# ethz-asl/voxgraph

Measured on AMD Instinct MI355X. Metric: Mresiduals+Jacobians/s per GPU; full pose-graph solve ms (200 submaps), higher is better.
Workload: dtype f32

## Files before the change

### profiles/fuzz_esdf.py

```python
#!/usr/bin/env python3
import os
import sys

import numpy as np

ROOT = os.path.dirname(os.path.dirname(os.path.abspath(__file__)))
sys.path.insert(0, ROOT)
F = np.float32
BAR = 4e-3


def main():
    from oracle import pyoracle as orc
    from oracle import synth
    from tests.test_esdf_gpu import _check_fixed_point
    from voxgraph_amd import capi
    capi.load()
    ctx = capi.Context(0)
    n_seeds, first = int(os.environ.get("SEEDS", "100")), int(os.environ.get("FIRST", "0"))
    done, worst, worst_fp, voxels, frontier = 0, 0.0, 0.0, 0, 0
    for seed in range(first, first + n_seeds):
        rng = np.random.default_rng(seed)
        vps = int(rng.choice([8, 16]))
        vs = float(rng.choice([0.05, 0.1, 0.2]))
        dims = tuple(int(x) for x in rng.integers(1, 5, 3))
        ext = np.array(dims) * vps * vs
        c = rng.uniform(0.2, 0.8, 3) * ext
        sdf = synth.sphere_ground_sdf(tuple(c), float(rng.uniform(0.2, 0.6) * ext.min()), float(rng.uniform(0.1, 0.4) * ext[2]))
        sm = synth.make_submap(sdf, vs, vps, tuple(int(x) for x in rng.integers(-2, 2, 3)), dims, trunc=3 * vs, esdf_max=10 * vs,
                               drop_empty_blocks=bool(rng.integers(0, 2)))
        if len(sm.block_index) == 0:
            continue
        td = sm.tsdf_distance.copy()
        if rng.integers(0, 2):
            td = np.clip(td + rng.normal(0, 0.02 * vs, td.shape).astype(F), -3 * vs, 3 * vs).astype(F)
        tw = sm.tsdf_weight.copy()
        if rng.integers(0, 2):
            tw = np.where(rng.uniform(size=tw.shape) < 0.03, 0, tw).astype(F)
        max_d = float(rng.choice([2.0, 6 * vs, 12 * vs]))
        kw = dict(max_distance_m=max_d, default_distance_m=float(rng.choice([max_d, 2.0])), min_distance_m=float(rng.choice([0.2, vs, 2 * vs])))
        what = dict(seed=seed, vps=vps, vs=vs, dims=dims, blocks=len(sm.block_index), **kw)
        g = capi.Submap(ctx, 0, vs, vps, sm.block_index, td, tw, None, None)
        try:
            g.generate_esdf(capi.esdf_config(**kw))
            _, _, ed, eo = g.download_layers(vps)
            od, oo, _ = orc.esdf_from_tsdf(vs, vps, sm.block_index, td, tw, orc.esdf_config(**kw))
            assert np.array_equal(eo, oo), "observed masks"
            obs = oo.astype(bool)
            fixed = (tw >= 1e-6) & (np.abs(td) < kw["min_distance_m"])
            assert np.array_equal(ed[fixed], td[fixed]), "fixed band"
            assert np.array_equal(np.sign(ed[obs]), np.sign(td[obs])), "signs"
            if obs.any():
                a_d, a_o = np.abs(ed), np.abs(od)
                lo = kw["max_distance_m"] - BAR
                frontier_v = obs & (kw["default_distance_m"] > kw["max_distance_m"]) & ((a_d > lo) | (a_o > lo))
                assert np.all(np.minimum(a_d[frontier_v], a_o[frontier_v]) > lo - BAR), "a shell voxel on one side, an inner one on the other"
                frontier += int((frontier_v & (np.abs(ed - od) >= BAR)).sum())
                cmp_ = obs & ~frontier_v
                diff = np.abs(ed - od)[cmp_]
                assert diff.size == 0 or diff.max() < BAR, ("distance", float(diff.max()))
                assert np.all(np.abs(ed[cmp_]) <= np.abs(od[cmp_]) + 1e-6), "device above the queue's value"
                worst = max(worst, float(diff.max()) if diff.size else 0.0)
                try:
                    err, n_free = _check_fixed_point(sm.block_index, td, ed, eo, vs, vps, kw["min_distance_m"], kw["max_distance_m"],
                                                     kw["default_distance_m"])
                except ValueError:
                    err, n_free = 0.0, 0
                assert err < 1e-6, ("fixed point", err)
                worst_fp = max(worst_fp, err)
                voxels += int(obs.sum())
        except AssertionError as e:
            print("MISMATCH", what, str(e)[:300])
            return 1
        finally:
            g.destroy()
        done += 1
    print("no mismatch in %d submaps (%d observed voxels): worst |device - queue| %.2e m (bar %.1e), worst fixed-point residual %.1e; "
          "%d voxels of the shell beyond max_distance_m differ by more (default > max configurations only)" %
          (done, voxels, worst, BAR, worst_fp, frontier))
    ctx.close()
    return 0


if __name__ == "__main__":
    sys.exit(main())
```

### voxgraph_amd/csrc/vgx_context.hip

```cpp
#include <algorithm>
#include <atomic>
#include <cmath>
#include <cstring>
#include <numeric>

#include <cstdlib>

#include "vgx_internal.h"

namespace vgx {

static std::mutex g_err_mu;
static std::string g_global_error = "no error";

void set_global_error(const std::string& msg) {
  std::lock_guard<std::mutex> lk(g_err_mu);
  g_global_error = msg;
}

int set_error(vgx_ctx ctx, int code, const std::string& msg) {
  if (ctx) {
    std::lock_guard<std::mutex> lk(ctx->err_mu);
    ctx->last_error = msg;
  } else {
    set_global_error(msg);
  }
  return code;
}

template <int VPS, int LAYOUT>
__global__ __launch_bounds__(256) void brickify_kernel(
    const int32_t* __restrict__ block_index, const int32_t* __restrict__ lut,
    int3 lut_min, int3 lut_dim, const float* __restrict__ distance,
    const float* __restrict__ weight, const uint8_t* __restrict__ observed,
    float* __restrict__ bricks) {
  constexpr int CELLS = BrickLayout<VPS, LAYOUT>::cells;
  constexpr int VOX = VPS * VPS * VPS;
  const int b = blockIdx.x;
  const int bx = block_index[3 * b + 0] - lut_min.x;
  const int by = block_index[3 * b + 1] - lut_min.y;
  const int bz = block_index[3 * b + 2] - lut_min.z;
  float* out = bricks + (size_t)b * CELLS;
  for (int cell = threadIdx.x; cell < CELLS; cell += blockDim.x) {
    int cx, cy, cz;
    BrickLayout<VPS, LAYOUT>::decode(cell, cx, cy, cz);
    int ox = cx == VPS, oy = cy == VPS, oz = cz == VPS;
    int sx = bx + ox, sy = by + oy, sz = bz + oz;
    int slot = b;
    if (ox | oy | oz) {
      slot = -1;
      if (sx < lut_dim.x && sy < lut_dim.y && sz < lut_dim.z)
        slot = lut[sx + lut_dim.x * (sy + lut_dim.y * sz)];
    }
    float v = __builtin_nanf("");
    if (slot >= 0) {
      int vx = ox ? 0 : cx, vy = oy ? 0 : cy, vz = oz ? 0 : cz;
      size_t at = (size_t)slot * VOX + vx + VPS * (vy + VPS * vz);
      bool ok = weight ? (weight[at] > 0.0f) : (observed[at] != 0);
      if (ok) v = distance[at];
    }
    out[cell] = v;
  }
}

int launch_brickify(vgx_submap sm, int which) {
  vgx_ctx ctx = sm->ctx;
  const float* dist = which == 0 ? sm->d_tsdf_distance : sm->d_esdf_distance;
  const float* w = which == 0 ? sm->d_tsdf_weight.get() : nullptr;
  const uint8_t* obs = which == 0 ? nullptr : sm->d_esdf_observed.get();
  const int layout = ctx->brick_layout;
  const size_t cells = brick_cells(sm->vps, layout);
  if ((unsigned long long)sm->n_blocks * cells >= (1ull << 32))
    return set_error(ctx, VGX_ERR_UNSUPPORTED,
                     "submap too large for 32-bit brick addressing: " + std::to_string(sm->n_blocks) + " blocks x " +
                         std::to_string(cells) + " cells per brick");
  size_t bytes = (size_t)sm->n_blocks * cells * sizeof(float);
  VGX_HIP(ctx, sm->grid[which].d_bricks.alloc(bytes));
  sm->grid[which].layout = layout;
  int3 mn = make_int3(sm->lut_min[0], sm->lut_min[1], sm->lut_min[2]);
  int3 dm = make_int3(sm->lut_dim[0], sm->lut_dim[1], sm->lut_dim[2]);
  dispatch_brick(sm->vps, layout, [&](auto V, auto L) {
    hipLaunchKernelGGL((brickify_kernel<V(), L()>), dim3(sm->n_blocks), dim3(256), 0, ctx->stream, sm->d_block_index, sm->d_lut, mn, dm,
                       dist, w, obs, sm->grid[which].d_bricks);
  });
  VGX_HIP(ctx, hipGetLastError());
  sm->grid[which].present = true;
  return VGX_OK;
}

template <int VPS>
__global__ __launch_bounds__(256) void requad_kernel(const float* __restrict__ apron, float* __restrict__ quad) {
  constexpr int CA = BrickLayout<VPS, 0>::cells, CQ = BrickLayout<VPS, 1>::cells, B = VPS + 1;
  const float* in = apron + (size_t)blockIdx.x * CA;
  float* out = quad + (size_t)blockIdx.x * CQ;
  for (int i = threadIdx.x; i < CQ; i += blockDim.x) {
    int cx, cy, cz;
    BrickLayout<VPS, 1>::decode(i, cx, cy, cz);
    out[i] = in[cx + B * (cy + B * cz)];
  }
}

__global__ __launch_bounds__(64) void chunk_bounds_kernel(const float4* __restrict__ xyzd, long long n,
                                                         float4* __restrict__ bounds,
                                                         float* __restrict__ chunk_minmax) {
  const long long first = (long long)blockIdx.x * kChunkPoints;
  float mn[3] = {INFINITY, INFINITY, INFINITY}, mx[3] = {-INFINITY, -INFINITY, -INFINITY};
  for (long long i = first + threadIdx.x; i < first + kChunkPoints && i < n; i += 64) {
    float4 p = xyzd[i];
    mn[0] = fminf(mn[0], p.x); mx[0] = fmaxf(mx[0], p.x);
    mn[1] = fminf(mn[1], p.y); mx[1] = fmaxf(mx[1], p.y);
    mn[2] = fminf(mn[2], p.z); mx[2] = fmaxf(mx[2], p.z);
  }
#pragma unroll
  for (int a = 0; a < 3; ++a)
#pragma unroll
    for (int off = 32; off >= 1; off >>= 1) {
      mn[a] = fminf(mn[a], __shfl_xor(mn[a], off, 64));
      mx[a] = fmaxf(mx[a], __shfl_xor(mx[a], off, 64));
    }
  if (threadIdx.x == 0) {
    float hx = 0.5f * (mx[0] - mn[0]), hy = 0.5f * (mx[1] - mn[1]), hz = 0.5f * (mx[2] - mn[2]);
    float r = sqrtf(hx * hx + hy * hy + hz * hz) * 1.0001f + 1e-4f;
    bounds[blockIdx.x] = make_float4(0.5f * (mx[0] + mn[0]), 0.5f * (mx[1] + mn[1]),
                                     0.5f * (mx[2] + mn[2]), r);
#pragma unroll
    for (int a = 0; a < 3; ++a) {
      chunk_minmax[6 * blockIdx.x + a] = mn[a];
      chunk_minmax[6 * blockIdx.x + 3 + a] = mx[a];
    }
  }
// ... 154 lines not shown
  if (std::string(prop.gcnArchName).rfind("gfx950", 0) != 0)
    return set_error(nullptr, VGX_ERR_NO_DEVICE,
                     std::string("vgx_ctx_create: device is ") + prop.gcnArchName +
                         ", this library is built for gfx950 only");
  vgx_ctx ctx = new (std::nothrow) vgx_ctx_s();
  if (!ctx) return set_error(nullptr, VGX_ERR_NOMEM, "vgx_ctx_create: out of host memory");
  ctx->device = device;
  ctx->cu_count = prop.multiProcessorCount;
  int prio_least = 0, prio_greatest = 0;
  const bool use_prio = hipSetDevice(device) == hipSuccess &&
                        hipDeviceGetStreamPriorityRange(&prio_least, &prio_greatest) == hipSuccess;
  ctx->stream_priorities = use_prio && prio_least != prio_greatest;
  if (hipSetDevice(device) != hipSuccess ||
      hipStreamCreateWithPriority(&ctx->own_stream, hipStreamNonBlocking, ctx->stream_priorities ? prio_least : 0) != hipSuccess ||
      hipStreamCreateWithPriority(&ctx->tsdf_own_stream, hipStreamNonBlocking, ctx->stream_priorities ? prio_greatest : 0) != hipSuccess ||
      hipEventCreate(&ctx->ev_start) != hipSuccess ||
      hipEventCreate(&ctx->ev_stop) != hipSuccess ||
      hipEventCreate(&ctx->ev_tsdf_start) != hipSuccess ||
      hipEventCreate(&ctx->ev_tsdf_stop) != hipSuccess ||
      hipEventCreateWithFlags(&ctx->ev_handover, hipEventDisableTiming) != hipSuccess) {
    if (ctx->own_stream) (void)hipStreamDestroy(ctx->own_stream);
    if (ctx->tsdf_own_stream) (void)hipStreamDestroy(ctx->tsdf_own_stream);
    for (hipEvent_t ev : {ctx->ev_start, ctx->ev_stop, ctx->ev_tsdf_start, ctx->ev_tsdf_stop, ctx->ev_handover})
      if (ev) (void)hipEventDestroy(ev);
    delete ctx;
    return set_error(nullptr, VGX_ERR_HIP, "vgx_ctx_create: stream/event creation failed");
  }
  ctx->stream = ctx->own_stream;
  ctx->tsdf_stream = ctx->tsdf_own_stream;
  ctx->last_error = "no error";
  *out = ctx;
  return VGX_OK;
}

int vgx_ctx_destroy(vgx_ctx ctx) {
  if (!ctx) return VGX_ERR_INVALID;
  (void)hipSetDevice(ctx->device);
  (void)hipStreamSynchronize(ctx->stream);
  (void)hipStreamSynchronize(ctx->tsdf_stream);
  for (hipEvent_t ev : {ctx->ev_start, ctx->ev_stop, ctx->ev_tsdf_start, ctx->ev_tsdf_stop, ctx->ev_handover})
    if (ev) (void)hipEventDestroy(ev);
  for (int k = 0; k < Context::kEvalSlots; ++k) {
    Context::EvalSlot& sl = ctx->eval_slot[k];
    if (sl.stream) {
      (void)hipStreamSynchronize(sl.stream);
      (void)hipStreamDestroy(sl.stream);
    }
    if (sl.order) (void)hipEventDestroy(sl.order);
    sl.d_out.release();
    sl.d_raw.release();
    sl.h_raw.release();
    sl.h_out.release();
  }
  if (ctx->own_stream) (void)hipStreamDestroy(ctx->own_stream);
  if (ctx->tsdf_own_stream) (void)hipStreamDestroy(ctx->tsdf_own_stream);
  delete ctx;
  return VGX_OK;
}

const char* vgx_last_error(vgx_ctx ctx) {
  static thread_local std::string copy;
  if (ctx) {
    std::lock_guard<std::mutex> lk(ctx->err_mu);
    copy = ctx->last_error;
  } else {
    std::lock_guard<std::mutex> lk(g_err_mu);
    copy = g_global_error;
  }
  return copy.c_str();
}

int vgx_ctx_set_stream(vgx_ctx ctx, void* hip_stream) {
  if (!ctx) return VGX_ERR_INVALID;
  std::lock_guard<std::mutex> lk(ctx->mu);
  ctx->stream = hip_stream ? (hipStream_t)hip_stream : ctx->own_stream;
  return VGX_OK;
}

void* vgx_ctx_get_stream(vgx_ctx ctx) { return ctx ? (void*)ctx->stream : nullptr; }

int vgx_ctx_set_tsdf_stream(vgx_ctx ctx, void* hip_stream) {
  if (!ctx) return VGX_ERR_INVALID;
  std::lock_guard<std::mutex> lk(ctx->tsdf_mu);
  (void)hipSetDevice(ctx->device);
  (void)hipStreamSynchronize(ctx->tsdf_stream);
  ctx->tsdf_stream = hip_stream ? (hipStream_t)hip_stream : ctx->tsdf_own_stream;
  return VGX_OK;
}

void* vgx_ctx_get_tsdf_stream(vgx_ctx ctx) { return ctx ? (void*)ctx->tsdf_stream : nullptr; }

int vgx_ctx_set_brick_layout(vgx_ctx ctx, int32_t layout) {
  if (!ctx) return VGX_ERR_INVALID;
  if (layout != VGX_BRICKS_APRON && layout != VGX_BRICKS_QUAD)
    return set_error(ctx, VGX_ERR_INVALID, "vgx_ctx_set_brick_layout: unknown layout");
  std::lock_guard<std::mutex> lk(ctx->mu);
  ctx->brick_layout = layout;
  return VGX_OK;
}

int vgx_ctx_set_sampling_bricks(vgx_ctx ctx, int32_t mode) {
  if (!ctx) return VGX_ERR_INVALID;
  if (mode != VGX_SAMPLING_BRICKS_SAME && mode != VGX_SAMPLING_BRICKS_QUAD)
    return set_error(ctx, VGX_ERR_INVALID, "vgx_ctx_set_sampling_bricks: unknown mode");
  std::lock_guard<std::mutex> lk(ctx->mu);
  ctx->sampling_bricks = mode;
// ... 339 lines not shown
```

### voxgraph_amd/csrc/vgx_esdf.hip

```cpp
#include <cmath>
#include <vector>

#include "vgx_internal.h"

#pragma clang fp contract(off)

namespace vgx {

struct TsdfLayerDevView;

__global__ __launch_bounds__(256) void esdf_init_kernel(const float* __restrict__ tsdf_d,
                                                        const float* __restrict__ tsdf_w,
                                                        size_t n, float min_weight,
                                                        float min_distance, float default_distance,
                                                        float* __restrict__ esdf_d,
                                                        uint8_t* __restrict__ esdf_obs) {
  size_t i = (size_t)blockIdx.x * blockDim.x + threadIdx.x;
  if (i >= n) return;
  float w = tsdf_w[i], d = tsdf_d[i];
  if (w < min_weight) {
    esdf_d[i] = 0.0f;
    esdf_obs[i] = 0;
    return;
  }
  esdf_obs[i] = 1;
  if (fabsf(d) < min_distance) {
    esdf_d[i] = d;
  } else {
    float sgn = (float)((d > 0.0f) - (d < 0.0f));
    esdf_d[i] = sgn * default_distance;
  }
}

constexpr int kLocalSweeps = 6;

template <int VPS>
__global__ __launch_bounds__(256) void esdf_relax_kernel(
    const int32_t* __restrict__ block_index, const int32_t* __restrict__ lut, int3 lut_min,
    int3 lut_dim, const float* __restrict__ tsdf_d, const uint8_t* __restrict__ esdf_obs,
    float* __restrict__ esdf_d, float voxel_size, float min_distance, float max_distance,
    int* __restrict__ changed) {
  constexpr int T = VPS + 2;
  constexpr int VOX = VPS * VPS * VPS;
  __shared__ float tile[T * T * T];
  __shared__ int s_changed;
  const int b = blockIdx.x;
  const int bx = block_index[3 * b] - lut_min.x, by = block_index[3 * b + 1] - lut_min.y,
            bz = block_index[3 * b + 2] - lut_min.z;
  if (threadIdx.x == 0) s_changed = 0;
  for (int c = threadIdx.x; c < T * T * T; c += 256) {
    int tx = c % T, ty = (c / T) % T, tz = c / (T * T);
    int vx = tx - 1, vy = ty - 1, vz = tz - 1;
    int ox = vx < 0 ? -1 : (vx >= VPS ? 1 : 0), oy = vy < 0 ? -1 : (vy >= VPS ? 1 : 0),
        oz = vz < 0 ? -1 : (vz >= VPS ? 1 : 0);
    int slot = b;
    if (ox | oy | oz) {
      int sx = bx + ox, sy = by + oy, sz = bz + oz;
      slot = -1;
      if ((unsigned)sx < (unsigned)lut_dim.x && (unsigned)sy < (unsigned)lut_dim.y &&
          (unsigned)sz < (unsigned)lut_dim.z)
        slot = lut[sx + lut_dim.x * (sy + lut_dim.y * sz)];
    }
    float v = __builtin_nanf("");
    if (slot >= 0) {
      size_t at = (size_t)slot * VOX + (size_t)((vx - ox * VPS) + VPS * ((vy - oy * VPS) + VPS * (vz - oz * VPS)));
      if (esdf_obs[at]) v = esdf_d[at];
    }
    tile[c] = v;
  }
  __syncthreads();
  const float s1 = voxel_size, s2 = sqrtf(2.0f) * voxel_size, s3 = sqrtf(3.0f) * voxel_size;
  bool any_change = false;
  for (int sweep = 0; sweep < kLocalSweeps; ++sweep) {
    bool sweep_change = false;
    for (int v = threadIdx.x; v < VOX; v += 256) {
      int x = v % VPS, y = (v / VPS) % VPS, z = v / (VPS * VPS);
      int c = (x + 1) + T * ((y + 1) + T * (z + 1));
      float cur = tile[c];
      if (!(cur == cur)) continue;
      if (fabsf(tsdf_d[(size_t)b * VOX + v]) < min_distance) continue;
      float mag = fabsf(cur);
      float best = mag;
#pragma unroll
      for (int dz = -1; dz <= 1; ++dz)
#pragma unroll
        for (int dy = -1; dy <= 1; ++dy)
#pragma unroll
          for (int dx = -1; dx <= 1; ++dx) {
            if (dx == 0 && dy == 0 && dz == 0) continue;
            float n = tile[c + dx + T * (dy + T * dz)];
            int nz = (dx != 0) + (dy != 0) + (dz != 0);
            float step = nz == 1 ? s1 : (nz == 2 ? s2 : s3);
            bool same = (cur > 0.0f && n > 0.0f) || (cur < 0.0f && n < 0.0f);
            float cand = fabsf(n) + step;
            if (same && fabsf(n) < max_distance && cand < best) best = cand;
          }
      if (best < mag) {
        tile[c] = cur > 0.0f ? best : -best;
        sweep_change = true;
      }
    }
    any_change |= sweep_change;
    if (sweep_change) s_changed = 1;
    __syncthreads();
    int again = s_changed;
    __syncthreads();
    if (!again) break;
    if (threadIdx.x == 0) s_changed = 0;
    __syncthreads();
  }
  if (__syncthreads_or(any_change)) {
    for (int v = threadIdx.x; v < VOX; v += 256) {
      int x = v % VPS, y = (v / VPS) % VPS, z = v / (VPS * VPS);
      float val = tile[(x + 1) + T * ((y + 1) + T * (z + 1))];
      if (val == val) esdf_d[(size_t)b * VOX + v] = val;
    }
    if (threadIdx.x == 0) atomicExch(changed, 1);
  }
}

}

using namespace vgx;

extern "C" {

void vgx_esdf_config_default(vgx_esdf_config* c) {
  if (!c) return;
  c->max_distance_m = 2.0f;
  c->min_distance_m = 0.2f;
  c->default_distance_m = 2.0f;
  c->min_diff_m = 0.001f;
  c->min_weight = 1e-6f;
  c->num_buckets = 20;
}

int vgx_submap_generate_esdf(vgx_submap sm, const vgx_esdf_config* cfg_in, int32_t* sweeps_out) {
  if (!sm) return VGX_ERR_INVALID;
  vgx_ctx ctx = sm->ctx;
  std::lock_guard<std::mutex> lk(ctx->mu);
  vgx_esdf_config cfg;
  if (cfg_in) cfg = *cfg_in; else vgx_esdf_config_default(&cfg);
  if (sm->n_blocks > 0 && (!sm->d_tsdf_distance || !sm->d_tsdf_weight))
    return set_error(ctx, VGX_ERR_INVALID, "vgx_submap_generate_esdf: TSDF layer not resident");
  if (!(cfg.max_distance_m > 0) || !(cfg.min_distance_m >= 0) || !(cfg.default_distance_m > 0))
    return set_error(ctx, VGX_ERR_INVALID, "vgx_submap_generate_esdf: bad config");
  VGX_HIP(ctx, hipSetDevice(ctx->device));
  if (sweeps_out) *sweeps_out = 0;
  if (sm->n_blocks == 0) return VGX_OK;
  const size_t nvox = (size_t)sm->n_blocks * sm->vps * sm->vps * sm->vps;
  VGX_HIP(ctx, hipStreamSynchronize(ctx->stream));
  if (!sm->d_esdf_distance) VGX_HIP(ctx, sm->d_esdf_distance.alloc_n(nvox));
  if (!sm->d_esdf_observed) VGX_HIP(ctx, sm->d_esdf_observed.alloc_n(nvox));
  DeviceBuffer s_changed;
  VGX_HIP(ctx, s_changed.alloc(sizeof(int)));
  int* d_changed = s_changed.as<int>();
  hipLaunchKernelGGL(esdf_init_kernel, dim3((unsigned)((nvox + 255) / 256)), dim3(256), 0, ctx->stream,
                     sm->d_tsdf_distance, sm->d_tsdf_weight, nvox, cfg.min_weight, cfg.min_distance_m,
                     cfg.default_distance_m, sm->d_esdf_distance, sm->d_esdf_observed);
  int3 mn = make_int3(sm->lut_min[0], sm->lut_min[1], sm->lut_min[2]);
  int3 dm = make_int3(sm->lut_dim[0], sm->lut_dim[1], sm->lut_dim[2]);
  int passes = 0, rc = VGX_OK;
  const int max_passes = 8 + (int)std::ceil(cfg.max_distance_m / sm->voxel_size) * 2;
  while (passes < max_passes) {
    hipError_t e = hipMemsetAsync(d_changed, 0, sizeof(int), ctx->stream);
    if (e == hipSuccess) {
      if (sm->vps == 16)
        hipLaunchKernelGGL(esdf_relax_kernel<16>, dim3(sm->n_blocks), dim3(256), 0, ctx->stream,
                           sm->d_block_index, sm->d_lut, mn, dm, sm->d_tsdf_distance,
                           sm->d_esdf_observed, sm->d_esdf_distance, sm->voxel_size,
                           cfg.min_distance_m, cfg.max_distance_m, d_changed);
      else
        hipLaunchKernelGGL(esdf_relax_kernel<8>, dim3(sm->n_blocks), dim3(256), 0, ctx->stream,
                           sm->d_block_index, sm->d_lut, mn, dm, sm->d_tsdf_distance,
                           sm->d_esdf_observed, sm->d_esdf_distance, sm->voxel_size,
                           cfg.min_distance_m, cfg.max_distance_m, d_changed);
      e = hipGetLastError();
    }
    int h_changed = 0;
    if (e == hipSuccess) e = hipMemcpyAsync(&h_changed, d_changed, sizeof(int), hipMemcpyDeviceToHost, ctx->stream);
    if (e == hipSuccess) e = hipStreamSynchronize(ctx->stream);
    if (e != hipSuccess) {
      rc = set_error(ctx, VGX_ERR_HIP, std::string("vgx_submap_generate_esdf: ") + hipGetErrorString(e));
      break;
    }
    ++passes;
    if (!h_changed) break;
  }
  if (rc != VGX_OK) return rc;
  if (sweeps_out) *sweeps_out = passes;
  if (sm->grid[1].d_bricks) {
    sm->grid[1].d_bricks.release();
    sm->grid[1].present = false;
  }
  sm->grid[1].d_quad.release();
  return launch_brickify(sm, 1);
}

}
```

### voxgraph_amd/csrc/vgx_internal.h

```cpp
#ifndef VGX_INTERNAL_H_
#define VGX_INTERNAL_H_

#include <hip/hip_runtime.h>

#include <algorithm>
#include <atomic>
#include <cstdint>
#include <mutex>
#include <condition_variable>
#include <initializer_list>
#include <random>
#include <string>
#include <type_traits>
#include <utility>
#include <vector>

#include "voxgraph_amd.h"

namespace vgx {


template <int VPS, int LAYOUT>
struct BrickLayout {
  static_assert(LAYOUT == 0 || LAYOUT == 1, "apron (0) or quad (1) bricks");
// ... 207 lines not shown
  for (const DeviceBufferSize& g : group) g.buffer->release();
  hipError_t e = hipSuccess;
  for (const DeviceBufferSize& g : group)
    if (e == hipSuccess) e = g.buffer->alloc(g.bytes);
  if (e != hipSuccess)
    for (const DeviceBufferSize& g : group) g.buffer->release();
  return e;
}

template <class Call>
hipError_t temp_bytes(Call& call, size_t* bytes) {
  *bytes = 0;
  return call(nullptr, *bytes);
}
template <class Call>
hipError_t run_with_temp(DeviceBuffer& tmp, Call& call) {
  size_t bytes = 0;
  hipError_t e = temp_bytes(call, &bytes);
  if (e == hipSuccess) e = tmp.reserve(bytes, 8);
  if (e == hipSuccess) e = call(tmp.p, bytes);
  return e;
}

struct Context {
  int device = 0;
  hipStream_t own_stream = nullptr;
  hipStream_t stream = nullptr;
  hipEvent_t ev_start = nullptr, ev_stop = nullptr;
  std::mutex mu;
  hipStream_t tsdf_own_stream = nullptr;
  hipStream_t tsdf_stream = nullptr;
  bool stream_priorities = false;
  std::atomic<int> tsdf_integrators{0};
  hipEvent_t ev_tsdf_start = nullptr, ev_tsdf_stop = nullptr, ev_handover = nullptr;
  std::mutex tsdf_mu;
  std::mutex err_mu;
  std::string last_error;
  int cu_count = 256;
  int brick_layout = 0;
  int sampling_bricks = 1;
  struct EvalSlot {
    hipStream_t stream = nullptr;
    hipEvent_t order = nullptr;
    DeviceBuffer d_out;
    DeviceBuffer d_raw;
    PinnedBuffer h_raw;
    PinnedBuffer h_out;
    bool busy = false;
  };
  static constexpr int kEvalSlots = 8;
  static constexpr size_t kSmallOutputBytes = 1u << 20;
  EvalSlot eval_slot[kEvalSlots];
  std::condition_variable slot_free;
};

struct Mt19937 {
  static constexpr int kN = 624;
  uint32_t mt[kN];
  uint32_t idx = kN;
  Mt19937() { seed(5489u); }
  void seed(uint32_t s) {
    mt[0] = s;
    for (int i = 1; i < kN; ++i) mt[i] = 1812433253u * (mt[i - 1] ^ (mt[i - 1] >> 30)) + (uint32_t)i;
    idx = kN;
  }
  void twist() {
    for (int k = 0; k < kN; ++k) {
      uint32_t y = (mt[k] & 0x80000000u) | (mt[(k + 1) % kN] & 0x7fffffffu);
      mt[k] = mt[(k + 397) % kN] ^ (y >> 1) ^ ((y & 1u) ? 0x9908b0dfu : 0u);
    }
    idx = 0;
  }
  uint32_t operator()() {
    if (idx >= (uint32_t)kN) twist();
    uint32_t y = mt[idx++];
    y ^= y >> 11;
    y ^= (y << 7) & 0x9d2c5680u;
    y ^= (y << 15) & 0xefc60000u;
    y ^= y >> 18;
    return y;
  }
};
static_assert(sizeof(Mt19937) == 625 * 4, "Mt19937 is copied to the device as 625 words");

struct SamplerEngine {
  Mt19937 host;
  DeviceArray<uint32_t> d_state;
  bool on_device = false;
};

struct PointSet {
  int64_t n = 0;
  uint64_t version = 0;
  DeviceArray<float4> d_xyzd;
  DeviceArray<float> d_weight;
  DeviceArray<float4> d_chunk_bounds;
  float aabb_min[3] = {0, 0, 0}, aabb_max[3] = {0, 0, 0};
  double sum_weight = 0;
  bool present = false;
  std::vector<int64_t> order;
  std::vector<int32_t> inv_order;
  std::vector<double> cumulative_weight;
  DeviceArray<double> d_cumulative;
  int32_t search_buckets = 0;
  DeviceArray<int32_t> d_search_lut;
  DeviceArray<int32_t> d_inv_order;
// ... 127 lines not shown
  return origin + ((float)idx + 0.5f) * voxel_size;
}

#define VGX_HIP(ctx, call)                                                      \
  do {                                                                          \
    hipError_t e__ = (call);                                                    \
    if (e__ != hipSuccess)                                                      \
      return vgx::set_error((ctx), VGX_ERR_HIP,                                 \
                            std::string(#call) + ": " + hipGetErrorString(e__)); \
  } while (0)

inline int alloc_error(vgx_ctx ctx, hipError_t e, const char* what) {
  (void)hipGetLastError();
  return set_error(ctx, e == hipErrorOutOfMemory ? VGX_ERR_NOMEM : VGX_ERR_HIP, std::string(what) + ": " + hipGetErrorString(e));
}

inline int upload_new(vgx_ctx ctx, DeviceBuffer& buffer, const void* src, size_t bytes) {
  buffer.release();
  if (bytes == 0) return VGX_OK;
  VGX_HIP(ctx, buffer.alloc(bytes));
  VGX_HIP(ctx, hipMemcpy(buffer.p, src, bytes, hipMemcpyHostToDevice));
  return VGX_OK;
}

struct MeshView {
  vgx_ctx ctx;
  bool holds_mesh;
  bool has_colors;
  bool per_vertex;
  int64_t n_tris;
  const float* vertices;
  const float* normals;
  const uint32_t* colors;
};
std::mutex& mesh_mutex(vgx_mesh M);
MeshView mesh_view(vgx_mesh M);

struct EvalTotals {
  double sum;
  float max_abs, min_abs;
  long long n_eval, n_ign, n_non, n_err_blocks;
};
struct EvalDevice {
  DeviceBuffer slot, has, pos, part, tot, tmp, ed, es, ebi;
};
int eval_check(const char* fn, vgx_submap gt, vgx_submap test, int32_t layer, int32_t mode, const void* details);
int eval_enqueue(vgx_submap gt, vgx_submap test, int32_t layer, int32_t mode, bool want_index, bool want_distance, bool want_set,
                 EvalDevice& D);
void eval_details(const EvalTotals& tot, vgx_voxel_evaluation_details* details);

#ifndef VGX_TOOLING_LIBRARY
int launch_brickify(vgx_submap sm, int which);
int build_block_lut(vgx_submap sm);
#else
inline int launch_brickify(vgx_submap sm, int which);
inline int build_block_lut(vgx_submap sm);
#endif
int build_chunk_bounds(vgx_ctx ctx, PointSet& ps);
void reset_point_set(PointSet& ps);
int engine_to_host(vgx_ctx ctx, SamplerEngine& e);
int engine_to_device(vgx_ctx ctx, SamplerEngine& e);
void make_pose_pack(const double ref_pose[4], const double read_pose[4], PosePack* out);
std::vector<Tile> make_tiles(int32_t constraint, int64_t n, int tile_points);
constexpr int kBlockThreads = 256;
constexpr int kPointsPerThread = 4;
constexpr int kTilePoints = kBlockThreads * kPointsPerThread;
}

extern "C" {
VGX_API int vgx_internal_set_error(vgx_ctx ctx, int code, const char* msg);
VGX_API int vgx_internal_launch_brickify(vgx_submap sm, int which);
VGX_API int vgx_internal_build_block_lut(vgx_submap sm);
}
#ifdef VGX_TOOLING_LIBRARY
namespace vgx {
inline int set_error(vgx_ctx ctx, int code, const std::string& msg) { return vgx_internal_set_error(ctx, code, msg.c_str()); }
inline int launch_brickify(vgx_submap sm, int which) { return vgx_internal_launch_brickify(sm, which); }
inline int build_block_lut(vgx_submap sm) { return vgx_internal_build_block_lut(sm); }
}
#endif

#endif
```

Before: 130,100.

## Rework ESDF relaxation with block wake marks, batched passes and column sweeps

The ESDF relaxation kernel now tracks which blocks changed and marks only them and their neighbours for the next pass, so settled blocks exit early. The host queues several passes per synchronisation and reads per-pass counts instead of syncing after every pass. The kernel also switches to per-thread z-column sweeps with register-rolled neighbour planes and integer-keyed min comparisons, and brick buffers are reused instead of reallocated. This mainly speeds up the ESDF generation path; the pose-graph residual/Jacobian metric may be largely unaffected. It adds complexity and risks subtle correctness issues in mark bookkeeping and in the float-as-uint ordering.

After: 129,800. About the same (-0.2%).

```diff
diff --git a/profiles/esdf_bench.py b/profiles/esdf_bench.py
--- /dev/null
+++ b/profiles/esdf_bench.py
@@ -0,0 +1,115 @@
+import argparse
+import hashlib
+import json
+import os
+import sys
+import time
+
+import numpy as np
+
+ROOT = os.path.dirname(os.path.dirname(os.path.abspath(__file__)))
+sys.path.insert(0, ROOT)
+
+from voxgraph_amd import capi
+
+F = np.float32
+
+
+def city256(ctx):
+    pose = [0.0, 0.0, 0.0, np.random.default_rng(2).uniform(-0.1, 0.1)]
+    return capi.Submap.synth_city(ctx, 0, 0.2, 16, (-8, -8, -4), (16, 16, 16), 0.6, 2.0, 10.0, np.array(pose), 2)
+
+
+def config2(ctx):
+    import torch
+    from harness import pipeline
+    n_az, n_el, scans, vs = 1024, 64, 20, 0.2
+    poses = pipeline.session_sensor_poses(30, scans)
+    P = poses[0].copy()
+    P[2] = 0.0
+    pts = torch.empty((n_az * n_el, 3), dtype=torch.float32, device="cuda")
+    layer = capi.TsdfLayer(ctx, vs, 16)
+    for j in (0, scans - 1):
+        layer.reserve(pipeline._inv_compose(P, poses[j])[4:7], 16.0 + 0.6 + 2 * vs)
+    integ = capi.FastTsdfIntegrator(ctx, capi.voxgraph_tsdf_config(deterministic=1), layer)
+    for j in range(scans):
+        capi.synth_city_scan(ctx, poses[j], n_az, n_el, np.deg2rad(33.2), 40.0, 2, pts.data_ptr())
+        ctx.synchronize()
+        integ.integrate_device(pipeline._inv_compose(P, poses[j]), pts.data_ptr(), None, n_az * n_el)
+    ctx.synchronize()
+    sm = capi.Submap.from_tsdf_layer(ctx, layer, 0)
+    integ.destroy()
+    layer.destroy()
+    return sm
+
+
+def config1(ctx):
+    from oracle import synth
+    ref, _ = synth.config1_pair()
+    return capi.Submap(ctx, 0, ref.voxel_size, ref.vps, ref.block_index, ref.tsdf_distance, ref.tsdf_weight, None, None)
+
+
+def layer_hash(sm, h=None):
+    _, _, ed, eo = sm.download_layers(sm.vps)
+    h = hashlib.sha256() if h is None else h
+    h.update(ed.tobytes())
+    h.update(eo.tobytes())
+    return h
+
+
+def spread(ms):
+    return {"min": round(min(ms), 4), "median": round(float(np.median(ms)), 4), "max": round(max(ms), 4)}
+
+
+def main():
+    ap = argparse.ArgumentParser()
+    ap.add_argument("--reps", type=int, default=20)
+    ap.add_argument("--fuzz", type=int, default=0)
+    ap.add_argument("--loop", type=int, default=0)
+    ap.add_argument("--sizes", nargs="+", default=["city256", "config2", "config1"])
+    args = ap.parse_args()
+    ctx = capi.Context(0)
+    if args.loop:
+        sm = city256(ctx)
+        for _ in range(args.loop):
+            sm.generate_esdf()
+        ctx.synchronize()
+        sm.destroy()
+        ctx.close()
+        return
+    res = {"library": os.path.basename(capi.LIB_PATH), "reps": args.reps, "sizes": {}}
+    for name in args.sizes:
+        sm = {"city256": city256, "config2": config2, "config1": config1}[name](ctx)
+        for _ in range(3):
+            passes = sm.generate_esdf()
+        ev, wall = [], []
+        for _ in range(args.reps):
+            ctx.synchronize()
+            t = time.perf_counter()
+            ctx.timer_start()
+            sm.generate_esdf()
+            ev.append(ctx.timer_stop())
+            wall.append((time.perf_counter() - t) * 1e3)
+        res["sizes"][name] = {"blocks": int(sm.num_blocks()), "passes": int(passes), "event_ms": spread(ev), "wall_ms": spread(wall),
+                              "sha256": layer_hash(sm).hexdigest()}
+        sm.destroy()
+    if args.fuzz:
+        from profiles.fuzz_esdf import case
+        h, n = hashlib.sha256(), 0
+        for seed in range(args.fuzz):
+            made = case(seed)
+            if made is None:
+                continue
+            d, td, tw, kw = made
+            sm = capi.Submap(ctx, 0, d.voxel_size, d.vps, d.block_index, td, tw, None, None)
+            sm.generate_esdf(capi.esdf_config(**kw))
+            layer_hash(sm, h)
+            sm.destroy()
+            n += 1
+        res["fuzz"] = {"seeds": args.fuzz, "submaps": n, "sha256": h.hexdigest()}
+    ctx.close()
+    print(json.dumps(res))
+
+
+if __name__ == "__main__":
+    main()
diff --git a/profiles/fuzz_esdf.py b/profiles/fuzz_esdf.py
--- a/profiles/fuzz_esdf.py
+++ b/profiles/fuzz_esdf.py
@@ -10,6 +10,30 @@
 BAR = 4e-3
 
 
+def case(seed):
+    from oracle import synth
+    rng = np.random.default_rng(seed)
+    vps = int(rng.choice([8, 16]))
+    vs = float(rng.choice([0.05, 0.1, 0.2]))
+    dims = tuple(int(x) for x in rng.integers(1, 5, 3))
+    ext = np.array(dims) * vps * vs
+    c = rng.uniform(0.2, 0.8, 3) * ext
+    sdf = synth.sphere_ground_sdf(tuple(c), float(rng.uniform(0.2, 0.6) * ext.min()), float(rng.uniform(0.1, 0.4) * ext[2]))
+    sm = synth.make_submap(sdf, vs, vps, tuple(int(x) for x in rng.integers(-2, 2, 3)), dims, trunc=3 * vs, esdf_max=10 * vs,
+                           drop_empty_blocks=bool(rng.integers(0, 2)))
+    if len(sm.block_index) == 0:
+        return None
+    td = sm.tsdf_distance.copy()
+    if rng.integers(0, 2):
+        td = np.clip(td + rng.normal(0, 0.02 * vs, td.shape).astype(F), -3 * vs, 3 * vs).astype(F)
+    tw = sm.tsdf_weight.copy()
+    if rng.integers(0, 2):
+        tw = np.where(rng.uniform(size=tw.shape) < 0.03, 0, tw).astype(F)
+    max_d = float(rng.choice([2.0, 6 * vs, 12 * vs]))
+    kw = dict(max_distance_m=max_d, default_distance_m=float(rng.choice([max_d, 2.0])), min_distance_m=float(rng.choice([0.2, vs, 2 * vs])))
+    return sm, td, tw, kw
+
+
 def main():
     from oracle import pyoracle as orc
     from oracle import synth
@@ -20,26 +44,12 @@
     n_seeds, first = int(os.environ.get("SEEDS", "100")), int(os.environ.get("FIRST", "0"))
     done, worst, worst_fp, voxels, frontier = 0, 0.0, 0.0, 0, 0
     for seed in range(first, first + n_seeds):
-        rng = np.random.default_rng(seed)
-        vps = int(rng.choice([8, 16]))
-        vs = float(rng.choice([0.05, 0.1, 0.2]))
-        dims = tuple(int(x) for x in rng.integers(1, 5, 3))
-        ext = np.array(dims) * vps * vs
-        c = rng.uniform(0.2, 0.8, 3) * ext
-        sdf = synth.sphere_ground_sdf(tuple(c), float(rng.uniform(0.2, 0.6) * ext.min()), float(rng.uniform(0.1, 0.4) * ext[2]))
-        sm = synth.make_submap(sdf, vs, vps, tuple(int(x) for x in rng.integers(-2, 2, 3)), dims, trunc=3 * vs, esdf_max=10 * vs,
-                               drop_empty_blocks=bool(rng.integers(0, 2)))
-        if len(sm.block_index) == 0:
+        made = case(seed)
+        if made is None:
             continue
-        td = sm.tsdf_distance.copy()
-        if rng.integers(0, 2):
-            td = np.clip(td + rng.normal(0, 0.02 * vs, td.shape).astype(F), -3 * vs, 3 * vs).astype(F)
-        tw = sm.tsdf_weight.copy()
-        if rng.integers(0, 2):
-            tw = np.where(rng.uniform(size=tw.shape) < 0.03, 0, tw).astype(F)
-        max_d = float(rng.choice([2.0, 6 * vs, 12 * vs]))
-        kw = dict(max_distance_m=max_d, default_distance_m=float(rng.choice([max_d, 2.0])), min_distance_m=float(rng.choice([0.2, vs, 2 * vs])))
-        what = dict(seed=seed, vps=vps, vs=vs, dims=dims, blocks=len(sm.block_index), **kw)
+        sm, td, tw, kw = made
+        vs, vps = sm.voxel_size, sm.vps
+        what = dict(seed=seed, vps=vps, vs=vs, blocks=len(sm.block_index), **kw)
         g = capi.Submap(ctx, 0, vs, vps, sm.block_index, td, tw, None, None)
         try:
             g.generate_esdf(capi.esdf_config(**kw))
diff --git a/voxgraph_amd/csrc/vgx_context.hip b/voxgraph_amd/csrc/vgx_context.hip
--- a/voxgraph_amd/csrc/vgx_context.hip
+++ b/voxgraph_amd/csrc/vgx_context.hip
@@ -63,19 +63,29 @@
   }
 }
 
+int reserve_bricks(vgx_submap sm, int which) {
+  vgx_ctx ctx = sm->ctx;
+  const size_t cells = brick_cells(sm->vps, ctx->brick_layout);
+  if ((unsigned long long)sm->n_blocks * cells >= (1ull << 32))
+    return set_error(ctx, VGX_ERR_UNSUPPORTED,
+                     "submap too large for 32-bit brick addressing: " + std::to_string(sm->n_blocks) + " blocks x " +
+                         std::to_string(cells) + " cells per brick");
+  const size_t bytes = (size_t)sm->n_blocks * cells * sizeof(float);
+  if (sm->grid[which].d_bricks.bytes != bytes || !sm->grid[which].d_bricks) {
+    sm->grid[which].present = false;
+    VGX_HIP(ctx, sm->grid[which].d_bricks.alloc(bytes));
+  }
+  return VGX_OK;
+}
+
 int launch_brickify(vgx_submap sm, int which) {
   vgx_ctx ctx = sm->ctx;
   const float* dist = which == 0 ? sm->d_tsdf_distance : sm->d_esdf_distance;
   const float* w = which == 0 ? sm->d_tsdf_weight.get() : nullptr;
   const uint8_t* obs = which == 0 ? nullptr : sm->d_esdf_observed.get();
   const int layout = ctx->brick_layout;
-  const size_t cells = brick_cells(sm->vps, layout);
-  if ((unsigned long long)sm->n_blocks * cells >= (1ull << 32))
-    return set_error(ctx, VGX_ERR_UNSUPPORTED,
-                     "submap too large for 32-bit brick addressing: " + std::to_string(sm->n_blocks) + " blocks x " +
-                         std::to_string(cells) + " cells per brick");
-  size_t bytes = (size_t)sm->n_blocks * cells * sizeof(float);
-  VGX_HIP(ctx, sm->grid[which].d_bricks.alloc(bytes));
+  const int rc = reserve_bricks(sm, which);
+  if (rc != VGX_OK) return rc;
   sm->grid[which].layout = layout;
   int3 mn = make_int3(sm->lut_min[0], sm->lut_min[1], sm->lut_min[2]);
   int3 dm = make_int3(sm->lut_dim[0], sm->lut_dim[1], sm->lut_dim[2]);
@@ -336,6 +346,9 @@
     sl.h_raw.release();
     sl.h_out.release();
   }
+  ctx->d_esdf_marks.release();
+  ctx->d_esdf_counts.release();
+  ctx->h_esdf_counts.release();
   if (ctx->own_stream) (void)hipStreamDestroy(ctx->own_stream);
   if (ctx->tsdf_own_stream) (void)hipStreamDestroy(ctx->tsdf_own_stream);
   delete ctx;
diff --git a/voxgraph_amd/csrc/vgx_esdf.hip b/voxgraph_amd/csrc/vgx_esdf.hip
--- a/voxgraph_amd/csrc/vgx_esdf.hip
+++ b/voxgraph_amd/csrc/vgx_esdf.hip
@@ -33,90 +33,169 @@
 }
 
 constexpr int kLocalSweeps = 6;
+constexpr int kPassGroup = 4;
+
+__device__ __forceinline__ uint32_t esdf_key(uint32_t v, uint32_t sign) { return (v ^ sign) - 1u; }
+__device__ __forceinline__ uint32_t umin3(uint32_t a, uint32_t b, uint32_t c) { return min(min(a, b), c); }
 
 template <int VPS>
-__global__ __launch_bounds__(256) void esdf_relax_kernel(
+__global__ __launch_bounds__(256) __attribute__((amdgpu_waves_per_eu(6))) void esdf_relax_kernel(
     const int32_t* __restrict__ block_index, const int32_t* __restrict__ lut, int3 lut_min,
     int3 lut_dim, const float* __restrict__ tsdf_d, const uint8_t* __restrict__ esdf_obs,
     float* __restrict__ esdf_d, float voxel_size, float min_distance, float max_distance,
-    int* __restrict__ changed) {
+    int pass, uint8_t* __restrict__ marks_now, uint8_t* __restrict__ marks_next,
+    int32_t* __restrict__ counts) {
   constexpr int T = VPS + 2;
+  constexpr int P = T * T;
   constexpr int VOX = VPS * VPS * VPS;
-  __shared__ float tile[T * T * T];
-  __shared__ int s_changed;
+  constexpr int COLS = VPS * VPS;
+  constexpr int ZLEN = VPS / (256 / COLS);
+  static_assert(256 % COLS == 0 && ZLEN >= 1 && ZLEN * (256 / COLS) == VPS && ZLEN <= 32, "a column per thread or per few");
+  __shared__ uint32_t tile[T * T * T];
+  __shared__ int s_marked;
+  __shared__ uint32_t s_wake;
   const int b = blockIdx.x;
+  if (pass > 0) {
+    if (counts[2 * (pass - 1)] == 0) return;
+    if (threadIdx.x == 0) {
+      s_marked = marks_now[b];
+      if (s_marked) marks_now[b] = 0;
+    }
+    __syncthreads();
+    if (!s_marked) return;
+  }
+  if (threadIdx.x == 0) {
+    atomicAdd(&counts[2 * pass + 1], 1);
+    s_wake = 0;
+  }
   const int bx = block_index[3 * b] - lut_min.x, by = block_index[3 * b + 1] - lut_min.y,
             bz = block_index[3 * b + 2] - lut_min.z;
-  if (threadIdx.x == 0) s_changed = 0;
-  for (int c = threadIdx.x; c < T * T * T; c += 256) {
-    int tx = c % T, ty = (c / T) % T, tz = c / (T * T);
-    int vx = tx - 1, vy = ty - 1, vz = tz - 1;
-    int ox = vx < 0 ? -1 : (vx >= VPS ? 1 : 0), oy = vy < 0 ? -1 : (vy >= VPS ? 1 : 0),
-        oz = vz < 0 ? -1 : (vz >= VPS ? 1 : 0);
-    int slot = b;
-    if (ox | oy | oz) {
-      int sx = bx + ox, sy = by + oy, sz = bz + oz;
-      slot = -1;
-      if ((unsigned)sx < (unsigned)lut_dim.x && (unsigned)sy < (unsigned)lut_dim.y &&
-          (unsigned)sz < (unsigned)lut_dim.z)
-        slot = lut[sx + lut_dim.x * (sy + lut_dim.y * sz)];
-    }
-    float v = __builtin_nanf("");
-    if (slot >= 0) {
-      size_t at = (size_t)slot * VOX + (size_t)((vx - ox * VPS) + VPS * ((vy - oy * VPS) + VPS * (vz - oz * VPS)));
-      if (esdf_obs[at]) v = esdf_d[at];
-    }
-    tile[c] = v;
+  const int col = threadIdx.x % COLS, x = col % VPS, row = col / VPS;
+  const int y = VPS == 16 ? (row >> 1) + 8 * (row & 1) : row;
+  const int z0 = (threadIdx.x / COLS) * ZLEN;
+  const size_t v0 = (size_t)b * VOX + (size_t)(x + VPS * (y + VPS * z0));
+  uint32_t free_mask = 0;
+#pragma unroll
+  for (int k = 0; k < ZLEN; ++k)
+    if (!(fabsf(tsdf_d[v0 + (size_t)k * COLS]) < min_distance)) free_mask |= 1u << k;
+  const uint32_t nan_bits = __float_as_uint(__builtin_nanf(""));
+#pragma unroll
+  for (int j = 0; j < VOX / 256; ++j) {
+    const int i = (int)threadIdx.x + 256 * j;
+    const float d = esdf_d[(size_t)b * VOX + i];
+    const uint8_t o = esdf_obs[(size_t)b * VOX + i];
+    tile[(i % VPS + 1) + T * ((i / VPS) % VPS + 1 + T * (i / COLS + 1))] = o ? __float_as_uint(d) : nan_bits;
+  }
+  constexpr int HZ = 2 * T * T, HY = 2 * T * VPS, HALO = HZ + HY + 2 * COLS;
+  static_assert(VOX + HALO == T * T * T, "block + halo fill the tile");
+#pragma unroll
+  for (int j = 0; j < (HALO + 255) / 256; ++j) {
+    const int h = (int)threadIdx.x + 256 * j;
+    if (h < HALO) {
+      int tx, ty, tz;
+      if (h < HZ) {
+        tx = (h % P) % T, ty = (h % P) / T, tz = h / P ? T - 1 : 0;
+      } else if (h < HZ + HY) {
+        const int r = (h - HZ) % (T * VPS);
+        tx = r % T, tz = 1 + r / T, ty = (h - HZ) / (T * VPS) ? T - 1 : 0;
+      } else {
+        const int r = (h - HZ - HY) % COLS;
+        ty = 1 + r % VPS, tz = 1 + r / VPS, tx = (h - HZ - HY) / COLS ? T - 1 : 0;
+      }
+      const int vx = tx - 1, vy = ty - 1, vz = tz - 1;
+      const int ox = vx < 0 ? -1 : (vx >= VPS ? 1 : 0), oy = vy < 0 ? -1 : (vy >= VPS ? 1 : 0),
+                oz = vz < 0 ? -1 : (vz >= VPS ? 1 : 0);
+      const int sx = bx + ox, sy = by + oy, sz = bz + oz;
+      const bool inside = (unsigned)sx < (unsigned)lut_dim.x && (unsigned)sy < (unsigned)lut_dim.y &&
+                          (unsigned)sz < (unsigned)lut_dim.z;
+      const int slot = lut[inside ? sx + lut_dim.x * (sy + lut_dim.y * sz) : 0];
+      const bool there = inside && slot >= 0;
+      const size_t at = (size_t)(there ? slot : b) * VOX + (size_t)((vx - ox * VPS) + VPS * ((vy - oy * VPS) + VPS * (vz - oz * VPS)));
+      const float d = esdf_d[at];
+      const uint8_t o = esdf_obs[at];
+      tile[tx + T * (ty + T * tz)] = there && o ? __float_as_uint(d) : nan_bits;
+    }
   }
   __syncthreads();
   const float s1 = voxel_size, s2 = sqrtf(2.0f) * voxel_size, s3 = sqrtf(3.0f) * voxel_size;
-  bool any_change = false;
-  for (int sweep = 0; sweep < kLocalSweeps; ++sweep) {
-    bool sweep_change = false;
-    for (int v = threadIdx.x; v < VOX; v += 256) {
-      int x = v % VPS, y = (v / VPS) % VPS, z = v / (VPS * VPS);
-      int c = (x + 1) + T * ((y + 1) + T * (z + 1));
-      float cur = tile[c];
-      if (!(cur == cur)) continue;
-      if (fabsf(tsdf_d[(size_t)b * VOX + v]) < min_distance) continue;
-      float mag = fabsf(cur);
-      float best = mag;
-#pragma unroll
-      for (int dz = -1; dz <= 1; ++dz)
-#pragma unroll
-        for (int dy = -1; dy <= 1; ++dy)
-#pragma unroll
-          for (int dx = -1; dx <= 1; ++dx) {
-            if (dx == 0 && dy == 0 && dz == 0) continue;
-            float n = tile[c + dx + T * (dy + T * dz)];
-            int nz = (dx != 0) + (dy != 0) + (dz != 0);
-            float step = nz == 1 ? s1 : (nz == 2 ? s2 : s3);
-            bool same = (cur > 0.0f && n > 0.0f) || (cur < 0.0f && n < 0.0f);
-            float cand = fabsf(n) + step;
-            if (same && fabsf(n) < max_distance && cand < best) best = cand;
-          }
-      if (best < mag) {
-        tile[c] = cur > 0.0f ? best : -best;
-        sweep_change = true;
+  const uint32_t max_key = __float_as_uint(max_distance) - 1u;
+  const int c0 = (x + 1) + T * ((y + 1) + T * (z0 + 1));
+  uint32_t moved = 0;
+  bool block_change = false, settled = false;
+  for (int sweep = 0; sweep < kLocalSweeps && !settled; ++sweep) {
+    uint32_t sweep_moved = 0;
+    uint32_t lo[9], mid[9], hi[9];
+#pragma unroll
+    for (int j = 0; j < 9; ++j) {
+      const int at = c0 + (j % 3 - 1) + T * (j / 3 - 1);
+      lo[j] = tile[at - P];
+      mid[j] = tile[at];
+    }
+#pragma unroll
+    for (int k = 0; k < ZLEN; ++k) {
+      const int c = c0 + k * P;
+#pragma unroll
+      for (int j = 0; j < 9; ++j) hi[j] = tile[c + P + (j % 3 - 1) + T * (j / 3 - 1)];
+      const uint32_t cur = mid[4], mag = cur & 0x7fffffffu;
+      if (((free_mask >> k) & 1u) && mag - 1u < 0x7f800000u) {
+        const uint32_t sign = cur ^ mag;
+        const uint32_t face = min(umin3(esdf_key(mid[1], sign), esdf_key(mid[3], sign), esdf_key(mid[5], sign)),
+                                  umin3(esdf_key(mid[7], sign), esdf_key(lo[4], sign), esdf_key(hi[4], sign)));
+        const uint32_t edge =
+            umin3(umin3(esdf_key(mid[0], sign), esdf_key(mid[2], sign), esdf_key(mid[6], sign)),
+                  umin3(esdf_key(mid[8], sign), esdf_key(lo[1], sign), esdf_key(lo[3], sign)),
+                  min(umin3(esdf_key(lo[5], sign), esdf_key(lo[7], sign), esdf_key(hi[1], sign)),
+                      umin3(esdf_key(hi[3], sign), esdf_key(hi[5], sign), esdf_key(hi[7], sign))));
+        const uint32_t corner =
+            umin3(umin3(esdf_key(lo[0], sign), esdf_key(lo[2], sign), esdf_key(lo[6], sign)),
+                  umin3(esdf_key(lo[8], sign), esdf_key(hi[0], sign), esdf_key(hi[2], sign)),
+                  min(esdf_key(hi[6], sign), esdf_key(hi[8], sign)));
+        uint32_t best = mag;
+        if (face < max_key) best = min(best, __float_as_uint(__uint_as_float(face + 1u) + s1));
+        if (edge < max_key) best = min(best, __float_as_uint(__uint_as_float(edge + 1u) + s2));
+        if (corner < max_key) best = min(best, __float_as_uint(__uint_as_float(corner + 1u) + s3));
+        if (best < mag) {
+          mid[4] = best | sign;
+          tile[c] = mid[4];
+          sweep_moved |= 1u << k;
+        }
       }
-    }
-    any_change |= sweep_change;
-    if (sweep_change) s_changed = 1;
-    __syncthreads();
-    int again = s_changed;
-    __syncthreads();
-    if (!again) break;
-    if (threadIdx.x == 0) s_changed = 0;
-    __syncthreads();
-  }
-  if (__syncthreads_or(any_change)) {
-    for (int v = threadIdx.x; v < VOX; v += 256) {
-      int x = v % VPS, y = (v / VPS) % VPS, z = v / (VPS * VPS);
-      float val = tile[(x + 1) + T * ((y + 1) + T * (z + 1))];
-      if (val == val) esdf_d[(size_t)b * VOX + v] = val;
-    }
-    if (threadIdx.x == 0) atomicExch(changed, 1);
-  }
+#pragma unroll
+      for (int j = 0; j < 9; ++j) {
+        lo[j] = mid[j];
+        mid[j] = hi[j];
+      }
+    }
+    moved |= sweep_moved;
+    settled = !__syncthreads_or(sweep_moved != 0);
+    block_change |= !settled;
+  }
+  if (!block_change) return;
+  if (moved) {
+    const uint32_t xs = 2u | (x == 0 ? 1u : 0u) | (x == VPS - 1 ? 4u : 0u);
+    const uint32_t ys = 2u | (y == 0 ? 1u : 0u) | (y == VPS - 1 ? 4u : 0u);
+    const uint32_t zs = 2u | (z0 == 0 && (moved & 1u) ? 1u : 0u) | (z0 + ZLEN == VPS && ((moved >> (ZLEN - 1)) & 1u) ? 4u : 0u);
+    const uint32_t xy = (ys & 1u ? xs : 0u) | (ys & 2u ? xs << 3 : 0u) | (ys & 4u ? xs << 6 : 0u);
+    const uint32_t wake = ((zs & 1u ? xy : 0u) | (zs & 2u ? xy << 9 : 0u) | (zs & 4u ? xy << 18 : 0u)) & ~(1u << 13);
+    if (wake) atomicOr(&s_wake, wake);
+  }
+  if (!settled && threadIdx.x == 0) atomicOr(&s_wake, 1u << 13);
+#pragma unroll
+  for (int k = 0; k < ZLEN; ++k) {
+    const uint32_t val = tile[c0 + k * P];
+    if ((val & 0x7fffffffu) <= 0x7f800000u) esdf_d[v0 + (size_t)k * COLS] = __uint_as_float(val);
+  }
+  __syncthreads();
+  if (threadIdx.x < 27 && ((s_wake >> threadIdx.x) & 1u)) {
+    const int sx = bx + (int)(threadIdx.x % 3) - 1, sy = by + (int)(threadIdx.x / 3 % 3) - 1,
+              sz = bz + (int)(threadIdx.x / 9) - 1;
+    if ((unsigned)sx < (unsigned)lut_dim.x && (unsigned)sy < (unsigned)lut_dim.y &&
+        (unsigned)sz < (unsigned)lut_dim.z) {
+      const int slot = threadIdx.x == 13 ? b : lut[sx + lut_dim.x * (sy + lut_dim.y * sz)];
+      if (slot >= 0) marks_next[slot] = 1;
+    }
+  }
+  if (threadIdx.x == 64) atomicAdd(&counts[2 * pass], 1);
 }
 
 }
@@ -152,48 +231,55 @@
   VGX_HIP(ctx, hipStreamSynchronize(ctx->stream));
   if (!sm->d_esdf_distance) VGX_HIP(ctx, sm->d_esdf_distance.alloc_n(nvox));
   if (!sm->d_esdf_observed) VGX_HIP(ctx, sm->d_esdf_observed.alloc_n(nvox));
-  DeviceBuffer s_changed;
-  VGX_HIP(ctx, s_changed.alloc(sizeof(int)));
-  int* d_changed = s_changed.as<int>();
+  int3 mn = make_int3(sm->lut_min[0], sm->lut_min[1], sm->lut_min[2]);
+  int3 dm = make_int3(sm->lut_dim[0], sm->lut_dim[1], sm->lut_dim[2]);
+  const int max_passes = 8 + (int)std::ceil(cfg.max_distance_m / sm->voxel_size) * 2;
+  const size_t n_counts = 2 * (size_t)max_passes;
+  if (ctx->d_esdf_marks.bytes < 2 * (size_t)sm->n_blocks) {
+    VGX_HIP(ctx, ctx->d_esdf_marks.alloc_n(2 * ((size_t)sm->n_blocks + (size_t)sm->n_blocks / 4)));
+    VGX_HIP(ctx, hipMemsetAsync(ctx->d_esdf_marks, 0, ctx->d_esdf_marks.bytes, ctx->stream));
+  }
+  VGX_HIP(ctx, ctx->d_esdf_counts.reserve(n_counts * sizeof(int32_t)));
+  VGX_HIP(ctx, ctx->h_esdf_counts.reserve(n_counts * sizeof(int32_t)));
+  uint8_t* d_marks[2] = {ctx->d_esdf_marks.get(), ctx->d_esdf_marks.get() + ctx->d_esdf_marks.bytes / 2};
+  int32_t* d_counts = ctx->d_esdf_counts.get();
+  const int32_t* h_counts = ctx->h_esdf_counts.as<int32_t>();
+  sm->grid[1].present = false;
+  sm->grid[1].d_quad.release();
+  VGX_HIP(ctx, hipMemsetAsync(d_counts, 0, n_counts * sizeof(int32_t), ctx->stream));
   hipLaunchKernelGGL(esdf_init_kernel, dim3((unsigned)((nvox + 255) / 256)), dim3(256), 0, ctx->stream,
                      sm->d_tsdf_distance, sm->d_tsdf_weight, nvox, cfg.min_weight, cfg.min_distance_m,
                      cfg.default_distance_m, sm->d_esdf_distance, sm->d_esdf_observed);
-  int3 mn = make_int3(sm->lut_min[0], sm->lut_min[1], sm->lut_min[2]);
-  int3 dm = make_int3(sm->lut_dim[0], sm->lut_dim[1], sm->lut_dim[2]);
-  int passes = 0, rc = VGX_OK;
-  const int max_passes = 8 + (int)std::ceil(cfg.max_distance_m / sm->voxel_size) * 2;
-  while (passes < max_passes) {
-    hipError_t e = hipMemsetAsync(d_changed, 0, sizeof(int), ctx->stream);
-    if (e == hipSuccess) {
+  int passes = 0, queued = 0;
+  bool settled = false;
+  while (!settled && queued < max_passes) {
+    const int group = std::min(kPassGroup, max_passes - queued);
+    for (int pass = queued; pass < queued + group; ++pass) {
       if (sm->vps == 16)
         hipLaunchKernelGGL(esdf_relax_kernel<16>, dim3(sm->n_blocks), dim3(256), 0, ctx->stream,
                            sm->d_block_index, sm->d_lut, mn, dm, sm->d_tsdf_distance,
                            sm->d_esdf_observed, sm->d_esdf_distance, sm->voxel_size,
-                           cfg.min_distance_m, cfg.max_distance_m, d_changed);
+                           cfg.min_distance_m, cfg.max_distance_m, pass, d_marks[pass & 1],
+                           d_marks[(pass + 1) & 1], d_counts);
       else
         hipLaunchKernelGGL(esdf_relax_kernel<8>, dim3(sm->n_blocks), dim3(256), 0, ctx->stream,
                            sm->d_block_index, sm->d_lut, mn, dm, sm->d_tsdf_distance,
                            sm->d_esdf_observed, sm->d_esdf_distance, sm->voxel_size,
-                           cfg.min_distance_m, cfg.max_distance_m, d_changed);
-      e = hipGetLastError();
-    }
-    int h_changed = 0;
-    if (e == hipSuccess) e = hipMemcpyAsync(&h_changed, d_changed, sizeof(int), hipMemcpyDeviceToHost, ctx->stream);
-    if (e == hipSuccess) e = hipStreamSynchronize(ctx->stream);
-    if (e != hipSuccess) {
-      rc = set_error(ctx, VGX_ERR_HIP, std::string("vgx_submap_generate_esdf: ") + hipGetErrorString(e));
-      break;
-    }
-    ++passes;
-    if (!h_changed) break;
-  }
-  if (rc != VGX_OK) return rc;
+                           cfg.min_distance_m, cfg.max_distance_m, pass, d_marks[pass & 1],
+                           d_marks[(pass + 1) & 1], d_counts);
+    }
+    VGX_HIP(ctx, hipGetLastError());
+    if (queued == 0) {
+      const int rc = reserve_bricks(sm, 1);
+      if (rc != VGX_OK) return rc;
+    }
+    VGX_HIP(ctx, hipMemcpyAsync(ctx->h_esdf_counts.p, d_counts, n_counts * sizeof(int32_t), hipMemcpyDeviceToHost, ctx->stream));
+    VGX_HIP(ctx, hipStreamSynchronize(ctx->stream));
+    queued += group;
+    while (passes < queued && !settled) settled = h_counts[2 * passes++] == 0;
+  }
+  if (!settled) VGX_HIP(ctx, hipMemsetAsync(ctx->d_esdf_marks, 0, ctx->d_esdf_marks.bytes, ctx->stream));
   if (sweeps_out) *sweeps_out = passes;
-  if (sm->grid[1].d_bricks) {
-    sm->grid[1].d_bricks.release();
-    sm->grid[1].present = false;
-  }
-  sm->grid[1].d_quad.release();
   return launch_brickify(sm, 1);
 }
 
diff --git a/voxgraph_amd/csrc/vgx_internal.h b/voxgraph_amd/csrc/vgx_internal.h
--- a/voxgraph_amd/csrc/vgx_internal.h
+++ b/voxgraph_amd/csrc/vgx_internal.h
@@ -283,6 +283,9 @@
   static constexpr size_t kSmallOutputBytes = 1u << 20;
   EvalSlot eval_slot[kEvalSlots];
   std::condition_variable slot_free;
+  DeviceArray<uint8_t> d_esdf_marks;
+  DeviceArray<int32_t> d_esdf_counts;
+  PinnedBuffer h_esdf_counts;
 };
 
 struct Mt19937 {
@@ -516,6 +519,7 @@
 #ifndef VGX_TOOLING_LIBRARY
 int launch_brickify(vgx_submap sm, int which);
 int build_block_lut(vgx_submap sm);
+int reserve_bricks(vgx_submap sm, int which);
 #else
 inline int launch_brickify(vgx_submap sm, int which);
 inline int build_block_lut(vgx_submap sm);
```
